# CUHK-SE-Group/MicroRank

Measured on AMD Instinct MI355X. Metric: PageRank GTEPS + RCA windows ranked/sec at 1/2/4/8 MI355X; % HBM roofline, higher is better.
Workload: dtype f64

## Files before the change

### microrank_amd/csrc/mr_graph_build.hip

```cpp
#include <algorithm>
#include <cstring>
#include <vector>

#include "mr_detect_dev.h"
#include "mr_prim.h"
#include "mr_sort.h"

namespace {
constexpr int BT = 256;
constexpr int LDS_HIST = 8192;
constexpr int ESET = 1024;
constexpr uint64_t EMPTY = ~0ull;

__device__ __forceinline__ uint64_t hmix(uint64_t z) {
    z ^= z >> 33;
    z *= 0xff51afd7ed558ccdull;
    z ^= z >> 33;
    z *= 0xc4ceb9fe1a85ec53ull;
    return z ^ (z >> 33);
}

__global__ void k_count_codes(const int64_t* span, int64_t S, int32_t* cnt) {
    int64_t i = (int64_t)blockIdx.x * blockDim.x + threadIdx.x;
    if (i < S) atomicAdd(&cnt[span[i]], 1);
// ... 1814 lines not shown
        }
    }
    if (i < w.n_po) {
        const int32_t t = w.po_tr[i], op = w.po_op[i];
        const int sd = side_of(w.state[t]);
        if (sd >= 0) w.o.g[sd].rs_ops[w.x.g[sd].zoff[t] + (i - w.po_off[t])] = w.o.g[sd].node_of_code[op];
    }
}

int mr_ix_launch2_batch(mr_ctx* ctx, int n, const mr_spans* const* sps, uint8_t* const* d_states, mr_graph* const* g0s,
                        mr_graph* const* g1s, IxBuild* const* b0s, IxBuild* const* b1s, int64_t* const* d_outs,
                        const DetIn* dets, bool fuse) {
    if (n < 1 || n > IXW || getenv("MR_NO_IX2") != nullptr) return MR_ERR_STATE;
    for (int k = 0; k < n; ++k) {
        const mr_spans* sp = sps[k];
        if (!sp->ekey.p || sp->n_podops > NS_PMAX || 2 * (3 * (int64_t)sp->n_podops + sp->n_edge_keys) > IX_LDS_WORDS)
            return MR_ERR_STATE;
    }
    hipStream_t st = ctx->stream;
    IxBatch<IxWinSel> as{};
    IxBatch<IxWinStats> at{};
    const char* ee = getenv("MR_IX_EPT");
    const int ept = ee ? std::max(1, atoi(ee)) : IX_EPT;
    IxBatch<IxWinCross> ac{};
    IxBatch<IxWinNodes> an{};
    IxBatch<IxWinTraces> ar{};
    as.n = at.n = ac.n = an.n = ar.n = n;
    int32_t bs = 0, bt = 0, bc = 0, br = 0;
    size_t lds = 4;
    int64_t words = 0;
    std::vector<int64_t> woff((size_t)n);
    const int TP = fuse ? DB : SEL_TILE;
    for (int k = 0; k < n; ++k) {
        const mr_spans* sp = sps[k];
        const int32_t NT = sp->n_traces, NP = sp->n_podops;
        const int64_t nek = sp->n_edge_keys;
        IxSide2 xs;
        NsArgs2 na;
        TrOut2 to;
        IxBuild* b[2] = {b0s[k], b1s[k]};
        mr_graph* g[2] = {g0s[k], g1s[k]};
        for (int j = 0; j < 2; ++j) {
            IxBuild& B = *b[j];
            mr_graph* G = g[j];
            B.dense = true;
            B.small = true;
            B.ecap = (uint64_t)nek;
            B.gkp = sp->ekey.p;
            MR_TRY(B.tflag.alloc(ctx, std::max(NT, 1)));
            MR_TRY(B.tpos.alloc(ctx, (size_t)NT + 1));
            MR_TRY(B.zoff.alloc(ctx, (size_t)NT + 1));
            MR_TRY(B.ocnt.alloc(ctx, std::max(NP, 1)));
            MR_TRY(B.ofirst.alloc(ctx, std::max(NP, 1)));
            MR_TRY(B.ocov.alloc(ctx, std::max(NP, 1)));
            MR_TRY(B.gc.alloc(ctx, (size_t)std::max<int64_t>(nek, 1)));
            MR_TRY(B.node_of_code.alloc(ctx, std::max(NP, 1)));
            MR_TRY(G->node_podop.alloc(ctx, std::max(NP, 1)));
            MR_TRY(G->len_o.alloc(ctx, std::max(NP, 1)));
            MR_TRY(G->nchild.alloc(ctx, std::max(NP, 1)));
            MR_TRY(G->cov.alloc(ctx, std::max(NP, 1)));
            MR_TRY(G->ss_par.alloc(ctx, NS_EMAX));
            MR_TRY(G->ss_off.alloc(ctx, (size_t)NP + 1));
            MR_TRY(G->trace_code.alloc(ctx, std::max(NT, 1)));
            MR_TRY(G->len_t.alloc(ctx, std::max(NT, 1)));
            MR_TRY(G->rs_ops.alloc(ctx, (size_t)std::max<int64_t>(sp->n_po, 1)));
            MR_TRY(G->rs_off.alloc(ctx, (size_t)NT + 1));
            xs.g[j] = IxSide{B.tflag.p, B.ocnt.p, B.ofirst.p, B.ocov.p, B.tpos.p, B.zoff.p, B.gc.p};
            na.g[j] = NsArgs{B.gc.p, B.ocnt.p, B.ofirst.p, B.ocov.p, B.node_of_code.p, G->node_podop.p, G->len_o.p,
                             G->nchild.p, G->cov.p, G->ss_par.p, G->ss_off.p, B.tpos.p + NT, B.zoff.p + NT, G->rs_off.p,
                             d_outs[k] + 8 * j, nullptr, nullptr};
            to.g[j] = TrOut{G->trace_code.p, G->len_t.p, G->rs_ops.p, G->rs_off.p, B.node_of_code.p};
        }
        const int32_t nt = (int32_t)std::max<int64_t>(cdiv((int64_t)NT, TP), 1);
        woff[(size_t)k] = words;
        words += 4 * (int64_t)nt;
        as.b0[k] = bs;
        bs += nt;
        as.w[k] = IxWinSel{dets ? dets[k] : DetIn{}, d_states[k], sp->tlen.p, sp->po_off.p, nullptr, nek, NT, NP, xs};
        at.b0[k] = bt;
        const int64_t ne = std::max(sp->n_po, sp->n_ed);
        const int ek = ee ? ept : ne >= IX_EPT_BIG ? IX_EPT_BATCH : IX_EPT;
        if (NT) bt += std::max(1, std::min(256, cdiv(ne, (int64_t)IX_BT * ek)));
        lds = std::max(lds, 2 * (3 * (size_t)NP + (size_t)nek) * sizeof(int32_t));
        at.w[k] = IxWinStats{d_states[k], sp->po_tr.p, sp->po_op.p, sp->po_cnt.p, sp->po_first.p, sp->ed_tr.p, sp->ed_eid.p,
                             sp->ed_cnt.p, sp->n_po, sp->n_ed, NP, (int32_t)nek, xs};
        ac.b0[k] = bc;
        bc += (int32_t)cdiv(sp->n_xj, 256);
        ac.w[k] = IxWinCross{d_states[k], sp->xj_tc.p, sp->xj_tp.p, sp->xj_eid.p, sp->n_xj, xs};
        an.b0[k] = 2 * k;
        an.w[k] = IxWinNodes{sp->ekey.p, nek, NP, 0, na};
        ar.b0[k] = br;
        if (NT || sp->n_po) br += (int32_t)cdiv(std::max<int64_t>(NT, sp->n_po), 256);
        ar.w[k] = IxWinTraces{d_states[k], sp->tlen.p, sp->po_tr.p, sp->po_op.p, sp->po_off.p, sp->n_po, NT, 0, xs, to};
    }
    for (int k = n; k <= IXW; ++k) {
        if (k <= IXW) {
            as.b0[k] = bs;
            at.b0[k] = bt;
            ac.b0[k] = bc;
            an.b0[k] = 2 * n;
            ar.b0[k] = br;
        }
    }
    unsigned long long* dst = nullptr;
    uint64_t epoch = 0;
    MR_TRY(mr_dl_status(ctx, words, &dst, &epoch));
    for (int k = 0; k < n; ++k) as.w[k].st = dst + woff[(size_t)k];
    if (fuse) {
        hipLaunchKernelGGL(k_ix_detect_scan2_b, dim3(bs), dim3(DB), 0, st, as, epoch);
    } else {
        if (dets) {
            int32_t bd = 0;
            IxBatch<IxWinSel> ad = as;
            for (int k = 0; k < n; ++k) {
                ad.b0[k] = bd;
                bd += (int32_t)cdiv((int64_t)sps[k]->n_traces, DB);
            }
            for (int k = n; k <= IXW; ++k) ad.b0[k] = bd;
            if (bd) hipLaunchKernelGGL(k_ix_detect_b, dim3(bd), dim3(DB), 0, st, ad);
        }
        hipLaunchKernelGGL(k_ix_sel_scan2_b, dim3(bs), dim3(SEL_T), 0, st, as, epoch);
    }
    if (bt) hipLaunchKernelGGL(k_ix_stats2_b, dim3(bt), dim3(IX_BT), lds, st, at);
    if (bc) hipLaunchKernelGGL(k_ix_cross2_b, dim3(bc), dim3(256), 0, st, ac);
    hipLaunchKernelGGL(k_nodes_small2_b, dim3(2 * n), dim3(NS_T), 0, st, an);
    if (br) hipLaunchKernelGGL(k_ix_traces2_b, dim3(br), dim3(256), 0, st, ar);
    MR_TRY_HIP(ctx, hipGetLastError());
    return MR_OK;
}

constexpr int LB_T = 512;
constexpr int64_t LB_LDS_WORDS = 30720;
constexpr int32_t LB_A3MAX = 4096;
bool mr_lo_fits(const mr_spans* sp) {
    return sp->indexed && sp->ekey.p && sp->n_podops <= NS_PMAX && sp->n_edge_keys <= NS_EMAX &&
           2 * (3 * (int64_t)sp->n_podops + sp->n_edge_keys) + 2 * (int64_t)sp->n_svcops <= LB_LDS_WORDS &&
           sp->n_svcops <= LB_A3MAX && sp->n_traces <= (1 << 24);
}
struct IxWinLoB {
    const int32_t *lo_tr, *lo_len, *lo_kid, *lo_first, *bstart;
    const int64_t *lo_off, *lsv_off, *le_off;
    const uint16_t *lo16, *lo_cnt;
    const uint32_t *lsv, *le;
    const long long *lo_ts, *lo_te, *lo_mx;
    const double* a3;
    const uint8_t* a3v;
    int64_t t0, t1;
    uint8_t* state;
    int8_t* side;
    unsigned long long* counts;
    int32_t NT, NP, nek, nsvc;
    uint32_t* kcnt[2];
    int64_t* tot[2];
    uint32_t* rows;
};
__host__ __device__ __forceinline__ size_t lo_region0(size_t gbytes) {
    return 2 * gbytes > (size_t)2048 * 8 ? 2 * gbytes : (size_t)2048 * 8;
}
constexpr int LB_R = 4;
__device__ __forceinline__ int32_t lo_trace_of(uint32_t e, uint32_t n, const uint32_t* st, int32_t nt) {
    if (n > 0) return (int32_t)(e / n);
    int32_t lo = 0;
#pragma unroll
    for (int32_t step = LO_BT_MAX / 2; step >= 1; step >>= 1) {
        const int32_t mid = lo + step;
        lo = mid < nt && st[mid] <= e ? mid : lo;
    }
    return lo;
}
__global__ void __launch_bounds__(LB_T, 6) k_lo_build_b(IxBatch<IxWinLoB> a) {
    extern __shared__ __attribute__((aligned(16))) unsigned char lraw[];
    __shared__ uint32_t pst[LO_BT_MAX + 1], est[LO_BT_MAX + 1];
    __shared__ int8_t ss[LO_BT_MAX];
    __shared__ unsigned long long bc[5][LB_T / WAVE];
    const int k = ixb_pick(a.b0, a.n);
    const IxWinLoB& w = a.w[k];
    const int32_t blk = (int32_t)blockIdx.x - a.b0[k];
    const int tid = threadIdx.x, lane = tid & (WAVE - 1), wv = tid / WAVE;
    const int32_t NP = w.NP, nek = w.nek;
    const size_t gbytes = ((size_t)NP * 12 + (size_t)nek * 4 + 15) / 16 * 16;
    const size_t reg0 = lo_region0(gbytes);
    double* la3 = (double*)(lraw + reg0);
    double* prod = (double*)lraw;
    const uint32_t cap = (uint32_t)(reg0 / 8 / LB_T * LB_T);
    for (int32_t c = tid; c < w.nsvc; c += LB_T) la3[c] = w.a3v[c] ? w.a3[c] : 0.0;
    const int32_t T0 = w.bstart[blk], nt = w.bstart[blk + 1] - T0;
    const int64_t P0 = w.lo_off[T0], Q0 = w.le_off[T0], V0 = w.lsv_off[T0];
    const uint32_t np = (uint32_t)(w.lo_off[T0 + nt] - P0), nq = (uint32_t)(w.le_off[T0 + nt] - Q0);
    const uint32_t nv = (uint32_t)(w.lsv_off[T0 + nt] - V0);
    if (tid == 0) {
        pst[nt] = np;
        est[nt] = nq;
    }
    constexpr int NS = LO_BT_MAX / LB_T;
    uint32_t va[NS], vb[NS];
    bool act[NS];
    double expect[NS];
    long long mx[NS];
    unsigned long long rows = 0;
#pragma unroll
    for (int q = 0; q < NS; ++q) {
        const int32_t t = q * LB_T + tid;
        const bool valid = t < nt;
        const int64_t i = (int64_t)T0 + (valid ? t : nt - 1);
        const int32_t len = w.lo_len[i];
        const long long ts = w.lo_ts[i], te = w.lo_te[i];
        mx[q] = w.lo_mx[i];
        va[q] = (uint32_t)(w.lsv_off[i] - V0);
        vb[q] = (uint32_t)(w.lsv_off[i + 1] - V0);
        const bool in = valid && len > 0 && ts >= w.t0 && te <= w.t1;
        rows += in ? (unsigned long long)len : 0ull;
        act[q] = in && mx[q] > 0;
        expect[q] = 0.0;
    }
    __syncthreads();
    for (uint32_t r0 = 0; r0 < nv; r0 += cap) {
        const uint32_t rn = min(cap, nv - r0);
        constexpr int LU = 8;
        for (uint32_t x0 = 0; x0 < rn; x0 += LU * LB_T) {
            uint32_t v[LU];
#pragma unroll
            for (int u = 0; u < LU; ++u) {
                const uint32_t x = x0 + (uint32_t)(u * LB_T + tid);
                v[u] = w.lsv[V0 + (int64_t)(r0 + min(x, rn - 1))];
            }
#pragma unroll
            for (int u = 0; u < LU; ++u) {
                const uint32_t x = x0 + (uint32_t)(u * LB_T + tid);
                if (x < rn) prod[x] = (double)(v[u] >> 16) * la3[v[u] & 0xffffu];
            }
        }
        __syncthreads();
#pragma unroll
        for (int q = 0; q < NS; ++q)
            if (act[q]) {
                const uint32_t lo = max(va[q], r0), hi = min(vb[q], r0 + rn);
                for (uint32_t j = lo; j < hi; j += 8) {
                    double p8[8];
#pragma unroll
                    for (int u = 0; u < 8; ++u) p8[u] = prod[min(j + u, hi - 1) - r0];
#pragma unroll
                    for (int u = 0; u < 8; ++u)
                        if (j + u < hi) expect[q] += p8[u];
                }
            }
        __syncthreads();
    }
    for (size_t x = (size_t)tid * 4; x < reg0; x += (size_t)LB_T * 4) *(uint32_t*)(lraw + x) = 0u;
    unsigned long long nab = 0, nno = 0, nz0 = 0, nz1 = 0;
#pragma unroll
    for (int q = 0; q < NS; ++q) {
        const int32_t t = q * LB_T + tid;
        const bool valid = t < nt;
        const int64_t i = (int64_t)T0 + (valid ? t : nt - 1);
        const int32_t kid0 = w.lo_kid[i], tr = w.lo_tr[i];
        const int64_t pa = w.lo_off[i], pb = w.lo_off[i + 1], ea = w.le_off[i];
        const int stt = act[q] ? ((double)mx[q] / 1000.0 > expect[q] ? 2 : 1) : 0;
        const int s_ = valid ? (stt == 2 ? 0 : stt == 1 ? 1 : -1) : -1;
        if (valid) {
            w.state[tr] = (uint8_t)stt;
            w.side[i] = (int8_t)s_;
            ss[t] = (int8_t)s_;
            pst[t] = (uint32_t)(pa - P0);
            est[t] = (uint32_t)(ea - Q0);
        }
        nab += stt == 2;
        nno += stt == 1;
        if (s_ == 0) nz0 += (unsigned long long)(pb - pa);
        else if (s_ == 1) nz1 += (unsigned long long)(pb - pa);
        const int kid = valid ? kid0 : -1;
        const int kp = __shfl_up(kid, 1, WAVE);
        const bool hd = kid >= 0 && (lane == 0 || kp != kid);
        const unsigned long long H = __ballot(hd), B0 = __ballot(s_ == 0), B1 = __ballot(s_ == 1);
        if (hd) {
            const unsigned long long above = lane == WAVE - 1 ? 0ull : H & (~0ull << (lane + 1));
            const unsigned long long run = (above ? (above & (0ull - above)) - 1ull : ~0ull) & (~0ull << lane);
            const uint32_t c0 = (uint32_t)__popcll(B0 & run), c1 = (uint32_t)__popcll(B1 & run);
            if (c0) atomicAdd(&w.kcnt[0][kid], c0);
            if (c1) atomicAdd(&w.kcnt[1][kid], c1);
        }
    }
    __syncthreads();
    constexpr int LB_LANE = 8;
    const bool lanewise = nt > 0 && pst[nt] - pst[nt - 1] <= (uint32_t)LB_LANE;
    if (lanewise) {
#pragma unroll
        for (int q = 0; q < NS; ++q) {
            const int32_t t = q * LB_T + tid;
            const int sd = t < nt ? (int)ss[t] : -1;
            if (sd < 0) continue;
            unsigned char* G = lraw + (size_t)sd * gbytes;
            const uint32_t a0 = pst[t], n = pst[t + 1] - a0, rot = n ? (uint32_t)t % n : 0u;
            uint32_t pc[LB_LANE];
            int32_t fr[LB_LANE];
#pragma unroll
            for (int u = 0; u < LB_LANE; ++u) {
                const uint32_t j = (uint32_t)u + rot;
                const int64_t e = P0 + (int64_t)a0 + (u < (int)n ? (j >= n ? j - n : j) : 0u);
                pc[u] = (uint32_t)w.lo16[e] | ((uint32_t)w.lo_cnt[e] << 16);
                fr[u] = w.lo_first[e];
            }
#pragma unroll
            for (int u = 0; u < LB_LANE; ++u)
                if (u < (int)n) {
                    const uint32_t c = pc[u] & 0xffffu;
                    atomicAdd((unsigned long long*)G + c, (unsigned long long)(pc[u] >> 16) | (1ull << 32));
                    atomicMax((int32_t*)(G + (size_t)NP * 8) + c, 0x7fffffff - fr[u]);
                }
            const uint32_t b0e = est[t], m = est[t + 1] - b0e, rte = m ? (uint32_t)t % m : 0u;
            uint32_t* Ge = (uint32_t*)(G + (size_t)NP * 12);
            for (uint32_t u0 = 0; u0 < m; u0 += LB_LANE) {
                uint32_t ev[LB_LANE];
#pragma unroll
                for (int u = 0; u < LB_LANE; ++u) {
                    const uint32_t j = u0 + (uint32_t)u, jr = j + rte;
                    ev[u] = w.le[Q0 + (int64_t)b0e + (j < m ? (jr >= m ? jr - m : jr) : 0u)];
                }
#pragma unroll
                for (int u = 0; u < LB_LANE; ++u)
                    if (u0 + (uint32_t)u < m) atomicAdd(Ge + (ev[u] & 0xffffu), ev[u] >> 16);
            }
        }
    }
    const uint32_t n0 = nt ? pst[1 < nt ? 1 : nt] - pst[0] : 0u;
    const uint32_t npo = n0 > 0 && np == (uint32_t)nt * n0 ? n0 : 0u;
    constexpr int NW = LB_T / WAVE;
    const uint32_t nmax = lanewise ? 0u : max(np, nq);
    for (uint32_t b0 = (uint32_t)wv * (LB_R * WAVE); b0 < nmax; b0 += NW * LB_R * WAVE) {
        uint32_t pc[LB_R], ev[LB_R];
        int32_t fr[LB_R];
#pragma unroll
        for (int r = 0; r < LB_R; ++r) {
            const uint32_t o = b0 + (uint32_t)(r * WAVE + lane);
            if (b0 < np) {
                const int64_t e = P0 + (int64_t)min(o, np - 1u);
                pc[r] = (uint32_t)w.lo16[e] | ((uint32_t)w.lo_cnt[e] << 16);
                fr[r] = w.lo_first[e];
            }
            if (b0 < nq) ev[r] = w.le[Q0 + (int64_t)min(o, nq - 1u)];
        }
#pragma unroll
        for (int r = 0; r < LB_R; ++r) {
            const uint32_t o = b0 + (uint32_t)(r * WAVE + lane);
            if (o < np) {
                const int sd = ss[lo_trace_of(o, npo, pst, nt)];
                if (sd >= 0) {
                    unsigned char* G = lraw + (size_t)sd * gbytes;
                    const uint32_t c = pc[r] & 0xffffu;
                    atomicAdd((unsigned long long*)G + c, (unsigned long long)(pc[r] >> 16) | (1ull << 32));
                    atomicMax((int32_t*)(G + (size_t)NP * 8) + c, 0x7fffffff - fr[r]);
                }
            }
            if (o < nq) {
                const int sd = ss[lo_trace_of(o, 0u, est, nt)];
                if (sd >= 0)
                    atomicAdd((uint32_t*)(lraw + (size_t)sd * gbytes + (size_t)NP * 12) + (ev[r] & 0xffffu), ev[r] >> 16);
            }
        }
    }
    __syncthreads();
    {
        unsigned long long v[5] = {nab, nno, rows, nz0, nz1};
#pragma unroll
        for (int m = 32; m >= 1; m >>= 1)
#pragma unroll
            for (int q = 0; q < 5; ++q) v[q] += __shfl_xor(v[q], m, WAVE);
        if (lane == 0)
#pragma unroll
            for (int q = 0; q < 5; ++q) bc[q][wv] = v[q];
    }
    __syncthreads();
    if (tid < 5) {
        unsigned long long v = 0;
        for (int q = 0; q < NW; ++q) v += bc[tid][q];
        if (v) {
            if (tid < 3) atomicAdd(&w.counts[(size_t)(blk % CSH) * 3 + tid], v);
            else atomicAdd((unsigned long long*)&w.tot[tid - 3][1], v);
        }
    }
    const size_t rw = 3 * (size_t)NP + (size_t)nek;
    uint32_t* R = w.rows + (size_t)blk * 2 * rw;
    for (int g = 0; g < 2; ++g) {
        const unsigned char* G = lraw + (size_t)g * gbytes;
        uint32_t* Rg = R + (size_t)g * rw;
        for (int32_t c = tid; c < NP; c += LB_T) {
            const unsigned long long v = ((const unsigned long long*)G)[c];
            Rg[c] = (uint32_t)v;
            Rg[NP + c] = (uint32_t)(v >> 32);
            Rg[2 * NP + c] = ((const uint32_t*)(G + (size_t)NP * 8))[c];
        }
        for (int32_t x = tid; x < nek; x += LB_T) Rg[3 * NP + x] = ((const uint32_t*)(G + (size_t)NP * 12))[x];
    }
    __syncthreads();
}
constexpr int LP_T = 256, LP_I = 16, LP_TILE = LP_T * LP_I;
struct IxWinLoPos {
    const int8_t* side;
    int32_t NT, pad_;
    unsigned long long* st;
    int32_t* pinv[2];
    int64_t* tot[2];
};
__global__ void __launch_bounds__(LP_T) k_lo_pos_b(IxBatch<IxWinLoPos> a, uint64_t epoch) {
    __shared__ int32_t sa[2][LP_T];
    __shared__ int32_t ex[2];
    __shared__ int32_t so[2][LP_TILE];
    const int k = ixb_pick(a.b0, a.n);
    const IxWinLoPos& w = a.w[k];
    const int32_t blk = (int32_t)blockIdx.x - a.b0[k], nblk = a.b0[k + 1] - a.b0[k];
    const int tid = threadIdx.x, lane = tid & (WAVE - 1);
    const int64_t base = (int64_t)blk * LP_TILE + (int64_t)tid * LP_I;
    int8_t sd[LP_I];
    if (base + LP_I <= w.NT) {
        const uint4 v = *(const uint4*)(w.side + base);
        memcpy(sd, &v, 16);
    } else {
#pragma unroll
        for (int q = 0; q < LP_I; ++q) sd[q] = base + q < w.NT ? w.side[base + q] : (int8_t)-1;
    }
    int32_t c0 = 0, c1 = 0;
#pragma unroll
    for (int q = 0; q < LP_I; ++q) {
        c0 += sd[q] == 0;
        c1 += sd[q] == 1;
    }
    sa[0][tid] = c0;
    sa[1][tid] = c1;
    __syncthreads();
    for (int o = 1; o < LP_T; o <<= 1) {
        const int32_t v0 = tid >= o ? sa[0][tid - o] : 0, v1 = tid >= o ? sa[1][tid - o] : 0;
        __syncthreads();
        sa[0][tid] += v0;
        sa[1][tid] += v1;
        __syncthreads();
    }
    if (tid < 2 * WAVE) {
        const int g = tid / WAVE;
        const int32_t agg = sa[g][LP_T - 1];
        const int64_t e = dl_lookback_wave(w.st + (size_t)g * nblk, blk, agg, epoch);
        if (lane == 0) {
            ex[g] = (int32_t)e;
            if (blk == nblk - 1) w.tot[g][0] = e + agg;
        }
    }
    int32_t r0 = sa[0][tid] - c0, r1 = sa[1][tid] - c1;
#pragma unroll
    for (int q = 0; q < LP_I; ++q) {
        const int32_t ix = (int32_t)(base + q);
        if (sd[q] == 0) so[0][r0++] = ix;
        else if (sd[q] == 1) so[1][r1++] = ix;
    }
    __syncthreads();
    for (int g = 0; g < 2; ++g) {
        const int32_t n = sa[g][LP_T - 1], e = ex[g];
        for (int32_t x = tid; x < n; x += LP_T) w.pinv[g][e + x] = so[g][x];
    }
}
struct IxLoRed {
    const uint32_t* rows;
    int32_t nblk, NP, nek, pad_;
    int32_t *ocnt[2], *ofinv[2], *ocov[2];
    uint32_t* gc[2];
};
__global__ void __launch_bounds__(256) k_lo_reduce_b(IxBatch<IxLoRed> a) {
    const int k = ixb_pick(a.b0, a.n);
    const IxLoRed& w = a.w[k];
    const int64_t rw = 3 * (int64_t)w.NP + w.nek;
    const int64_t col = (int64_t)((int32_t)blockIdx.x - a.b0[k]) * 256 + threadIdx.x;
    if (col >= 2 * rw) return;
    const int g = (int)(col / rw);
    const int64_t c = col - (int64_t)g * rw;
    const bool mx = c >= 2 * (int64_t)w.NP && c < 3 * (int64_t)w.NP;
    const uint32_t* p = w.rows + col;
    const size_t stride = 2 * (size_t)rw;
    uint32_t acc = 0;
    int32_t b = 0;
    for (; b + 8 <= w.nblk; b += 8) {
        uint32_t v[8];
#pragma unroll
        for (int q = 0; q < 8; ++q) v[q] = p[(size_t)(b + q) * stride];
#pragma unroll
        for (int q = 0; q < 8; ++q) acc = mx ? max(acc, v[q]) : acc + v[q];
    }
    for (; b < w.nblk; ++b) {
        const uint32_t v = p[(size_t)b * stride];
        acc = mx ? max(acc, v) : acc + v;
    }
    const int32_t NP = w.NP;
    if (c < NP) w.ocnt[g][c] = (int32_t)acc;
    else if (c < 2 * (int64_t)NP) w.ocov[g][c - NP] = (int32_t)acc;
    else if (c < 3 * (int64_t)NP) w.ofinv[g][c - 2 * NP] = (int32_t)acc;
    else w.gc[g][c - 3 * NP] = acc;
}

int64_t mr_lo_zero_words(const mr_spans* sp) {
    return 2 * ((int64_t)std::max(sp->lo_nk, 1) + 3 * (int64_t)sp->n_podops + std::max<int64_t>(sp->n_edge_keys, 1));
}
int mr_lo_launch_batch(mr_ctx* ctx, int n, const mr_spans* const* sps, mr_graph* const* g0s, mr_graph* const* g1s,
                       IxBuild* const* b0s, IxBuild* const* b1s, int64_t* const* d_outs, const DetIn* dets,
                       uint32_t* const* zw) {
    if (n < 1 || n > IXW || getenv("MR_NO_IX2") != nullptr) return MR_ERR_STATE;
    for (int k = 0; k < n; ++k)
        if (!sps[k]->lo_ok || !mr_lo_fits(sps[k])) return MR_ERR_STATE;
    hipStream_t st = ctx->stream;
    IxBatch<IxWinLoB> ab{};
    IxBatch<IxLoRed> ar{};
    IxBatch<IxWinLoPos> ap{};
    IxBatch<IxWinCross> ac{};
    IxBatch<IxWinNodes> an{};
    ab.n = ar.n = ap.n = ac.n = an.n = n;
    int32_t bb = 0, bc = 0, br = 0, bp = 0;
    int64_t rwords = 0, sbytes = 0;
    std::vector<int64_t> roff((size_t)n), soff((size_t)n);
    size_t lds = 4;
    int64_t words = 0;
    std::vector<int64_t> woff((size_t)n);
    for (int k = 0; k < n; ++k) {
        const mr_spans* sp = sps[k];
        const int32_t NT = sp->n_traces, NP = sp->n_podops;
        const int64_t nek = sp->n_edge_keys, nk = std::max(sp->lo_nk, 1);
        IxSide2 xs;
        NsArgs2 na;
        IxBuild* b[2] = {b0s[k], b1s[k]};
        mr_graph* g[2] = {g0s[k], g1s[k]};
        IxWinLoB& L = ab.w[k];
        const int64_t per = nk + 3 * (int64_t)NP + std::max<int64_t>(nek, 1);
        for (int j = 0; j < 2; ++j) {
            IxBuild& B = *b[j];
            mr_graph* G = g[j];
            B.dense = true;
            B.small = true;
            B.ecap = (uint64_t)nek;
            B.gkp = sp->ekey.p;
            uint32_t* z = zw[k] + j * per;
            B.kcnt = z;
            int32_t* ocnt = (int32_t*)(z + nk);
            int32_t* ofinv = ocnt + NP;
            int32_t* ocov = ofinv + NP;
            uint32_t* gc = (uint32_t*)(ocov + NP);
            MR_TRY(B.pinv.alloc(ctx, std::max(NT, 1)));
            MR_TRY(B.node_of_code.alloc(ctx, std::max(NP, 1)));
            MR_TRY(G->node_podop.alloc(ctx, std::max(NP, 1)));
            MR_TRY(G->len_o.alloc(ctx, std::max(NP, 1)));
            MR_TRY(G->nchild.alloc(ctx, std::max(NP, 1)));
            MR_TRY(G->cov.alloc(ctx, std::max(NP, 1)));
            MR_TRY(G->u_o.alloc(ctx, std::max(NP, 1)));
            MR_TRY(G->pw.alloc(ctx, std::max(NP, 1)));
            MR_TRY(G->ss_par.alloc(ctx, NS_EMAX));
            MR_TRY(G->ss_off.alloc(ctx, (size_t)NP + 1));
            xs.g[j] = IxSide{nullptr, ocnt, ofinv, ocov, nullptr, nullptr, gc};
            int64_t* out = d_outs[k] + 8 * j;
            na.g[j] = NsArgs{gc, ocnt, ofinv, ocov, B.node_of_code.p, G->node_podop.p, G->len_o.p, G->nchild.p, G->cov.p,
                             G->ss_par.p, G->ss_off.p, out + 5, out + 6, nullptr, out, G->u_o.p, G->pw.p, 1};
            ap.w[k].pinv[j] = B.pinv.p;
            ap.w[k].tot[j] = out + 5;
            L.kcnt[j] = B.kcnt;
            L.tot[j] = out + 5;
            IxLoRed& R = ar.w[k];
            R.ocnt[j] = ocnt;
            R.ofinv[j] = ofinv;
            R.ocov[j] = ocov;
            R.gc[j] = gc;
        }
        const int32_t nt = sp->lo_nblk;
        const int64_t rw = 3 * (int64_t)NP + nek;
        roff[(size_t)k] = rwords;
        rwords += (int64_t)nt * 2 * rw;
        ar.w[k].nblk = nt;
        ar.w[k].NP = NP;
        ar.w[k].nek = (int32_t)nek;
        ar.b0[k] = br;
        br += (int32_t)cdiv(2 * rw, 256);
        const int32_t npb = (int32_t)std::max<int64_t>(cdiv((int64_t)NT, LP_TILE), 1);
        woff[(size_t)k] = words;
        words += 2 * (int64_t)npb;
        ap.b0[k] = bp;
        bp += npb;
        ap.w[k].NT = NT;
        soff[(size_t)k] = sbytes;
        sbytes += ((int64_t)NT + 15) / 16 * 16;
        ab.b0[k] = bb;
        bb += nt;
        const DetIn& d = dets[k];
        L.bstart = sp->lo_bstart.p;
        L.lo_tr = sp->lo_tr.p;
        L.lo_len = sp->lo_len.p;
        L.lo_kid = sp->lo_kid.p;
        L.lo_first = sp->lo_first.p;
        L.lo_off = sp->lo_off.p;
        L.lsv_off = sp->lsv_off.p;
        L.le_off = sp->le_off.p;
        L.lo16 = sp->lo16.p;
        L.lo_cnt = sp->lo_cnt.p;
        L.lsv = sp->lsv.p;
        L.le = sp->le.p;
        L.lo_ts = sp->lo_ts.p;
        L.lo_te = sp->lo_te.p;
        L.lo_mx = sp->lo_mx.p;
        L.a3 = d.a3;
        L.a3v = d.a3v;
        L.t0 = d.t0;
        L.t1 = d.t1;
        L.state = d.state;
        L.counts = d.counts;
        L.NT = NT;
        L.NP = NP;
        L.nek = (int32_t)nek;
        L.nsvc = sp->n_svcops;
        lds = std::max(lds, lo_region0(((size_t)NP * 12 + (size_t)nek * 4 + 15) / 16 * 16) + (size_t)sp->n_svcops * 8);
        ac.b0[k] = bc;
        bc += (int32_t)cdiv(sp->n_xj, 256);
        ac.w[k] = IxWinCross{d.state, sp->xj_tc.p, sp->xj_tp.p, sp->xj_eid.p, sp->n_xj, xs};
        an.b0[k] = 2 * k;
        an.w[k] = IxWinNodes{sp->ekey.p, nek, NP, 0, na};
    }
    for (int k = n; k <= IXW; ++k) {
        ab.b0[k] = bb;
        ar.b0[k] = br;
        ap.b0[k] = bp;
        ac.b0[k] = bc;
        an.b0[k] = 2 * n;
    }
    unsigned long long* dst = nullptr;
    uint64_t epoch = 0;
    MR_TRY(mr_dl_status(ctx, words, &dst, &epoch));
    DBuf<uint32_t> rows;
    DBuf<int8_t> side;
    MR_TRY(rows.alloc(ctx, (size_t)std::max<int64_t>(rwords, 1)));
    MR_TRY(side.alloc(ctx, (size_t)std::max<int64_t>(sbytes, 16)));
    for (int k = 0; k < n; ++k) {
        ab.w[k].rows = rows.p + roff[(size_t)k];
        ar.w[k].rows = rows.p + roff[(size_t)k];
        ab.w[k].side = side.p + soff[(size_t)k];
        ap.w[k].side = side.p + soff[(size_t)k];
        ap.w[k].st = dst + woff[(size_t)k];
    }
    hipLaunchKernelGGL(k_lo_build_b, dim3(bb), dim3(LB_T), lds, st, ab);
    hipLaunchKernelGGL(k_lo_pos_b, dim3(bp), dim3(LP_T), 0, st, ap, epoch);
    hipLaunchKernelGGL(k_lo_reduce_b, dim3(br), dim3(256), 0, st, ar);
    if (bc) hipLaunchKernelGGL(k_ix_cross2_b, dim3(bc), dim3(256), 0, st, ac);
    hipLaunchKernelGGL(k_nodes_small2_b, dim3(2 * n), dim3(NS_T), 0, st, an);
    MR_TRY_HIP(ctx, hipGetLastError());
    return MR_OK;
}

int mr_ix_launch(mr_ctx* ctx, const mr_spans* sp, const uint8_t* d_mask, mr_graph* g, IxBuild& b, int64_t* d_out) {
    return ix_launch(ctx, sp, d_mask, g, b, d_out, false);
}
int mr_ix_finish(mr_ctx* ctx, const mr_spans* sp, mr_graph* g, IxBuild& b, const int64_t* h) {
    MR_TRY(ix_finish(ctx, sp, g, b, h, false));
    return mr_graph_post_build(ctx, g);
}
int mr_ix_finish_unprepared(mr_ctx* ctx, const mr_spans* sp, mr_graph* g, IxBuild& b, const int64_t* h) {
    MR_TRY(ix_finish(ctx, sp, g, b, h, false));
    g->rs_is_sr = true;
    g->pr_identity = true;
    g->n_pr = g->T;
    return MR_OK;
}

int mr_graph_post_build(mr_ctx* ctx, mr_graph* g) {
    g->rs_is_sr = true;
    g->pr_identity = true;
    g->n_pr = g->T;
    PhaseTimer pt(ctx->stream, "prepare");
    MR_TRY(mr_graph_prepare(ctx, g));
    pt.mark("done");
    return MR_OK;
}

int mr_graph_build_dev(mr_ctx* ctx, const mr_spans* sp, const uint8_t* d_mask, mr_graph** out, const int64_t* win) {
    auto g = new mr_graph();
    g->ctx = ctx;
    static const bool no_index = getenv("MR_NO_INDEX") != nullptr;
    const bool indexed = sp->indexed && !no_index && (!win || sp->uniform_times);
    int rc = indexed ? graph_build_indexed(ctx, sp, d_mask, g) : graph_build_rows(ctx, sp, d_mask, win, g);
    if (rc == MR_OK) rc = mr_graph_post_build(ctx, g);
    if (rc != MR_OK) {
        delete g;
        return rc;
    }
    *out = g;
    return MR_OK;
}

extern "C" int mr_graph_build(mr_ctx* ctx, const mr_spans* sp, const uint8_t* trace_mask, mr_graph** out) {
    if (!ctx || !sp || !trace_mask || !out || sp->ctx != ctx) return mr_fail(ctx, MR_ERR_ARG, "mr_graph_build: bad arguments");
    MR_TRY_HIP(ctx, hipSetDevice(ctx->device));
    DBuf<uint8_t> mask;
    MR_TRY(mask.upload(ctx, trace_mask, (size_t)sp->n_traces));
    MR_TRY(mr_graph_build_dev(ctx, sp, mask.p, out, nullptr));
    mr_handle_add(ctx, *out, [](void* h) { delete (mr_graph*)h; });
    return MR_OK;
}

extern "C" int mr_graph_build_sharded(mr_ctx* ctx, const mr_spans* sp, const uint8_t* trace_mask, mr_graph** out) {
    if (!ctx || !sp || !trace_mask || !out || sp->ctx != ctx)
        return mr_fail(ctx, MR_ERR_ARG, "mr_graph_build_sharded: bad arguments");
    if (!mr_coll_ready(ctx) && ctx->nranks != 1) return mr_fail(ctx, MR_ERR_COMM, "no collective backend");
    if (!sp->indexed) return mr_fail(ctx, MR_ERR_STATE, "span table has no per-trace index (sharded build needs it)");
    MR_TRY_HIP(ctx, hipSetDevice(ctx->device));
    *out = nullptr;
    DBuf<uint8_t> mask;
    MR_TRY(mask.upload(ctx, trace_mask, (size_t)sp->n_traces));
    auto g = new mr_graph();
    g->ctx = ctx;
    int rc = graph_build_indexed(ctx, sp, mask.p, g, true);
    if (rc == MR_OK) {
        g->rs_is_sr = true;
        g->pr_identity = true;
        g->n_pr = g->T;
        rc = mr_graph_prepare(ctx, g);
    }
    if (rc == MR_OK) rc = hipStreamSynchronize(ctx->stream) == hipSuccess ? MR_OK : mr_fail(ctx, MR_ERR_HIP, "sync");
    if (rc != MR_OK) {
        delete g;
        return rc;
    }
    mr_handle_add(ctx, g, [](void* h) { delete (mr_graph*)h; });
    *out = g;
    return MR_OK;
}

extern "C" int mr_graph_nodes(const mr_graph* g, int32_t* node_podop, int32_t* trace_code) {
    if (!g) return MR_ERR_ARG;
    mr_ctx* ctx = g->ctx;
    if (!g->node_podop.p && g->N) return mr_fail(ctx, MR_ERR_STATE, "graph was not built from spans");
    if (node_podop && g->N) MR_TRY(g->node_podop.download(ctx, node_podop, g->N));
    if (trace_code && g->T) MR_TRY(g->trace_code.download(ctx, trace_code, g->T));
    MR_TRY_HIP(ctx, hipStreamSynchronize(ctx->stream));
    return MR_OK;
}

extern "C" int mr_graph_export(const mr_graph* g, int64_t* sr_off, int32_t* sr_ops, int32_t* len_t, int32_t* len_o,
                               int64_t* ss_off, int32_t* ss_par, int32_t* nchild) {
    if (!g) return MR_ERR_ARG;
    mr_ctx* ctx = g->ctx;
    if (sr_off) MR_TRY(g->rs_off.download(ctx, sr_off, (size_t)g->T + 1));
    if (sr_ops) MR_TRY(g->rs_ops.download(ctx, sr_ops, (size_t)g->nnz_rs));
    if (sr_ops) {
        std::vector<int64_t> off((size_t)g->T + 1);
        MR_TRY(g->rs_off.download(ctx, off.data(), off.size()));
        MR_TRY_HIP(ctx, hipStreamSynchronize(ctx->stream));
        for (int32_t t = 0; t < g->T; ++t) std::sort(sr_ops + off[t], sr_ops + off[t + 1]);
    }
    if (len_t) MR_TRY(g->len_t.download(ctx, len_t, (size_t)g->T));
    if (len_o) MR_TRY(g->len_o.download(ctx, len_o, (size_t)g->N));
    if (ss_off) MR_TRY(g->ss_off.download(ctx, ss_off, (size_t)g->N + 1));
    if (ss_par) MR_TRY(g->ss_par.download(ctx, ss_par, (size_t)g->E));
    if (nchild) MR_TRY(g->nchild.download(ctx, nchild, (size_t)g->N));
    MR_TRY_HIP(ctx, hipStreamSynchronize(ctx->stream));
    return MR_OK;
}
```

### microrank_amd/csrc/mr_pagerank.hip

```cpp
#include <algorithm>
#include <chrono>
#include <cmath>
#include <cstdlib>
#include <cstring>
#include <memory>
#include <queue>
#include <type_traits>

#include "mr_internal.h"
#include "mr_prim.h"
#include "mr_sort.h"

namespace {

constexpr int TB = 256;
constexpr int LDS_NODES = 8192;
constexpr int VCAP = 2048;
constexpr int LONG_PAIR = 32;
constexpr int TSHIFT_MIN = 8, TSHIFT_MAX = 12;

__device__ __forceinline__ uint64_t mix64(uint64_t z) {
    z += 0x9E3779B97F4A7C15ull;
    z = (z ^ (z >> 30)) * 0xBF58476D1CE4E5B9ull;
    z = (z ^ (z >> 27)) * 0x94D049BB133111EBull;
// ... 1253 lines not shown
    if (i < N) {
        G.sp0[i] = v0;
        G.su0[i] = (double)G.u_o[G.perm ? G.perm[i] : i] * v0;
    }
    if (i >= N && i < N + TR_PAD) G.su0[i] = G.su1[i] = 0.0;
    if (i < T) {
        const double q = (double)G.w_tq[i] * v0;
        if (G.fp32) G.q32[i] = (float)q; else G.q64[i] = q;
    }
    if (i < MSLOT_WORDS) G.mslot[i] = i < 2 * MSH ? d2bits(1.0) : 0ull;
}
__global__ void __launch_bounds__(KB) k_kind_insert_b(const SDev* __restrict__ sd, int32_t ng, uint64_t seed,
                                                      uint64_t hmask) {
    const SDev& G = sd[sd_graph(sd, ng, (int32_t)blockIdx.x, 1)];
    kind_insert_body<false, 2>((int32_t)blockIdx.x - G.b_kins, G.off, nullptr, G.o16, G.w_t, G.T, G.hk, G.cr,
                                  G.slot_of, (uint64_t)(G.cap - 1), seed, nullptr, hmask);
}
__global__ void k_kind_verify_b(const SDev* __restrict__ sd, int32_t ng) {
    const SDev& G = sd[sd_graph(sd, ng, (int32_t)blockIdx.x, 2)];
    const int32_t t = ((int32_t)blockIdx.x - G.b_kver) * blockDim.x + threadIdx.x;
    if (t >= G.T) return;
    const KCnt ks = G.cr[G.slot_of[t]];
    const int32_t r = ks.rep;
    G.kind[t] = (double)ks.cnt;
    if (r == t) return;
    const int64_t a0 = G.off[t], a1 = G.off[t + 1], b0 = G.off[r], b1 = G.off[r + 1];
    bool eq = (a1 - a0) == (b1 - b0);
    if (eq && a1 > a0) eq = __float_as_uint(G.w_t[t]) == __float_as_uint(G.w_t[r]);
    for (int64_t i = 0; eq && i < a1 - a0; ++i) eq = G.o16[a0 + i] == G.o16[b0 + i];
    if (!eq) atomicOr(G.flag, 1);
}
__global__ void k_pref_partial_b(const SDev* __restrict__ sd, int32_t ng) {
    __shared__ double red[TB / WAVE];
    const SDev& G = sd[sd_graph(sd, ng, (int32_t)blockIdx.x, 3)];
    const int32_t blk = (int32_t)blockIdx.x - G.b_pref;
    double a = 0.0, b = 0.0;
    const int32_t i = blk * blockDim.x + threadIdx.x;
    if (i < G.T) {
        const int32_t ln = G.len_t[i];
        a = 1.0 / G.kind[i];
        if (ln == 0) atomicOr(G.flag + 1, 1);
        b = ln ? 1.0 / (double)ln : 0.0;
    }
    a = block_sum(a, red);
    b = block_sum(b, red);
    if (threadIdx.x == 0) {
        G.ppart[2 * blk] = a;
        G.ppart[2 * blk + 1] = b;
    }
}
__global__ void k_pref_total_b(const SDev* __restrict__ sd) {
    __shared__ double red[1024 / WAVE];
    const SDev& G = sd[blockIdx.x];
    const int32_t nb = cdiv_d(G.T, TB);
    double a = 0.0, b = 0.0;
    for (int32_t i = threadIdx.x; i < nb; i += blockDim.x) {
        a += G.ppart[2 * i];
        b += G.ppart[2 * i + 1];
    }
    a = block_sum(a, red);
    b = block_sum(b, red);
    if (threadIdx.x == 0) {
        G.scal[2] = a;
        G.scal[3] = b;
    }
}
__global__ void k_pref_apply_b(const SDev* __restrict__ sd, int32_t ng) {
    const SDev& G = sd[sd_graph(sd, ng, (int32_t)blockIdx.x, 3)];
    const int32_t t = ((int32_t)blockIdx.x - G.b_pref) * blockDim.x + threadIdx.x;
    if (t >= G.T) return;
    const int32_t i = G.tpos[t];
    const double k = G.kind[t];
    double v;
    if (!G.anomaly) v = 1.0 / k / G.scal[2];
    else v = 1.0 / (k / G.scal[2] * G.phi + 1.0 / (double)G.len_t[t]) / G.scal[3] * G.phi;
    const float vf = (float)v;
    G.pref[t] = vf;
    G.c_t[t] = G.cd * vf;
    G.c_tp[i] = G.cd * vf;
}

constexpr int LO_NOC_MAX = 4096;
struct LDev {
    int32_t T, N, W, anomaly, fp32, NP;
    int32_t b_cs, n_cs, b_fill, nbp, b_app;
    int64_t st_off;
    float cd;
    double phi, v0;
    const int32_t* pinv;
    const int64_t* lo_off;
    const uint16_t* lo16;
    const int32_t *lo_len, *lo_kid, *noc;
    const uint32_t* kcnt;
    int64_t* c64;
    int32_t* coff;
    uint16_t* tids;
    float *w_tp, *c_tp;
    double* kind;
    int32_t* lenp;
    uint8_t* trun;
    double *ppart, *scal;
    int32_t* flag;
    unsigned long long* mslot;
    double *sp0, *su0, *su1, *q64;
    float* q32;
    const float* u_o;
};
__device__ __forceinline__ int32_t ld_graph(const LDev* ld, int32_t n, int32_t blk, int which) {
    int32_t lo = 0, hi = n - 1;
    while (lo < hi) {
        const int32_t mid = (lo + hi + 1) >> 1;
        const LDev& g = ld[mid];
        const int32_t s0 = which == 0 ? g.b_cs : which == 1 ? g.b_fill : g.b_app;
        if (s0 <= blk) lo = mid; else hi = mid - 1;
    }
    return lo;
}
__global__ void __launch_bounds__(TS_T) k_lo_cs_b(const LDev* __restrict__ ld, int32_t n, unsigned long long* st,
                                                 uint64_t epoch) {
    const LDev& G = ld[ld_graph(ld, n, (int32_t)blockIdx.x, 0)];
    tr_chunk_scan_body((int32_t)blockIdx.x - G.b_cs, G.n_cs, G.pinv, G.lo_off, G.T, G.W, G.c64, G.coff, st + G.st_off,
                       epoch);
}
__global__ void __launch_bounds__(256) k_lo_fill_b(const LDev* __restrict__ ld, int32_t n) {
    __shared__ double red[256 / WAVE];
    __shared__ uint16_t lnoc[LO_NOC_MAX];
    const LDev& G = ld[ld_graph(ld, n, (int32_t)blockIdx.x, 1)];
    const int32_t blk = (int32_t)blockIdx.x - G.b_fill;
    const int64_t i = (int64_t)blk * 256 + threadIdx.x;
    const int32_t T = G.T, N = G.N;
    for (int32_t c = threadIdx.x; c < G.NP; c += 256) lnoc[c] = (uint16_t)G.noc[c];
    __syncthreads();
    double a = 0.0, b = 0.0;
    if (i < (int64_t)G.W * WAVE) {
        const int32_t k = (int32_t)(i / WAVE), lane = (int32_t)(i % WAVE);
        int64_t e0 = 0, len = 0, rot = 0;
        const int32_t ix = i < T ? G.pinv[i] : -1;
        const int32_t kid = i < T ? G.lo_kid[ix] : -1;
        const int32_t kp = __shfl_up(kid, 1, WAVE);
        const bool hd = lane == 0 || kid < 0 || kid != kp;
        const unsigned long long hm = __ballot(hd);
        const unsigned long long below = hm & (lane == WAVE - 1 ? ~0ull : (2ull << lane) - 1ull);
        const int32_t ixh = __shfl(ix, 63 - __builtin_clzll(below), WAVE);
        const bool mt = G.trun && G.c64[k + 1] - G.c64[k] <= MR_TR_TIERS512;
        if (i < T && G.trun) {
            const unsigned long long above = lane == WAVE - 1 ? 0ull : hm & (~0ull << (lane + 1));
            G.trun[i] = !mt ? (uint8_t)1 : hd ? (uint8_t)((above ? __builtin_ctzll(above) : WAVE) - lane) : (uint8_t)0;
        }
        if (i < T) {
            e0 = G.lo_off[ix];
            len = G.lo_off[ix + 1] - e0;
            rot = len ? (int64_t)((uint32_t)(mt ? ixh : ix) % (uint32_t)len) : 0;
            const int32_t L = G.lo_len[ix];
            const uint32_t kc = G.kcnt[G.lo_kid[ix]];
            G.w_tp[i] = L > 0 ? (float)(1.0 / (double)L) : 0.0f;
            G.lenp[i] = L;
            G.kind[i] = (double)kc;
            a = 1.0 / (double)kc;
            b = L ? 1.0 / (double)L : 0.0;
        }
        const int64_t nc = G.c64[k + 1] - G.c64[k];
        unsigned long long* dst = (unsigned long long*)G.tids + (size_t)G.c64[k] * WAVE + lane;
        constexpr int TF_CH = 4;
        for (int64_t c0 = 0; c0 < nc; c0 += TF_CH) {
            uint16_t idv[4 * TF_CH];
#pragma unroll
            for (int q = 0; q < 4 * TF_CH; ++q) {
                const int64_t e = 4 * c0 + q, jx = rot + e;
                idv[q] = e < len ? lnoc[G.lo16[e0 + (jx >= len ? jx - len : jx)]] : (uint16_t)(N + lane);
            }
#pragma unroll
            for (int u = 0; u < TF_CH; ++u)
                if (c0 + u < nc)
                    dst[(size_t)(c0 + u) * WAVE] = (unsigned long long)idv[4 * u] | (unsigned long long)idv[4 * u + 1] << 16 |
                                                   (unsigned long long)idv[4 * u + 2] << 32 |
                                                   (unsigned long long)idv[4 * u + 3] << 48;
        }
    }
    a = block_sum(a, red);
    b = block_sum(b, red);
    if (threadIdx.x == 0) {
        G.ppart[2 * blk] = a;
        G.ppart[2 * blk + 1] = b;
    }
}
__global__ void __launch_bounds__(1024) k_lo_total_b(const LDev* __restrict__ ld) {
    __shared__ double red[1024 / WAVE];
    const LDev& G = ld[blockIdx.x];
    double a = 0.0, b = 0.0;
    for (int32_t i = threadIdx.x; i < G.nbp; i += blockDim.x) {
        a += G.ppart[2 * i];
        b += G.ppart[2 * i + 1];
    }
    a = block_sum(a, red);
    b = block_sum(b, red);
    if (threadIdx.x == 0) {
        G.scal[2] = a;
        G.scal[3] = b;
    }
}
__global__ void k_lo_apply_b(const LDev* __restrict__ ld, int32_t n) {
    const LDev& G = ld[ld_graph(ld, n, (int32_t)blockIdx.x, 2)];
    const int64_t i = (int64_t)((int32_t)blockIdx.x - G.b_app) * blockDim.x + threadIdx.x;
    const int32_t T = G.T, N = G.N;
    const double v0 = G.v0;
    if (i < T) {
        const double k = G.kind[i];
        double v;
        if (!G.anomaly) v = 1.0 / k / G.scal[2];
        else v = 1.0 / (k / G.scal[2] * G.phi + 1.0 / (double)G.lenp[i]) / G.scal[3] * G.phi;
        const float vf = (float)v;
        G.c_tp[i] = G.cd * vf;
        const double q = (double)G.w_tp[i] * v0;
        if (G.fp32) G.q32[i] = (float)q; else G.q64[i] = q;
    }
    if (i < N) {
        G.sp0[i] = v0;
        G.su0[i] = (double)G.u_o[i] * v0;
    }
    if (i >= N && i < N + TR_PAD) G.su0[i] = G.su1[i] = 0.0;
    if (i < MSLOT_WORDS) G.mslot[i] = i < 2 * MSH ? d2bits(1.0) : 0ull;
    if (i < 4) G.flag[i] = 0;
    if (i < 8 && i != 2 && i != 3) G.scal[i] = 0.0;
}

__global__ void k_iter_init(const float* w_t, const double* mw, const float* u_o, int32_t N, int32_t T, int64_t T_all,
                            double* sp0, double* su0, double* su1, double* q64, float* q32, int fp32,
                            unsigned long long* mslot, const int32_t* perm) {
    int64_t i = (int64_t)blockIdx.x * blockDim.x + threadIdx.x;
    const double v0 = 1.0 / (double)((int64_t)N + T_all);
    if (i < N) {
        sp0[i] = v0;
        su0[i] = (double)u_o[perm ? perm[i] : i] * v0;
    }
    if (i >= N && i < N + TR_PAD) su0[i] = su1[i] = 0.0;
    if (i < T) {
        double q = (mw ? mw[i] : (double)w_t[i]) * v0;
        if (fp32) q32[i] = (float)q; else q64[i] = q;
    }
    if (i < MSLOT_WORDS) mslot[i] = i < 2 * MSH ? d2bits(1.0) : 0ull;
}
__global__ void k_pr_reset_init(int32_t T, int64_t cap, int32_t N, float* pref, float* c_t, unsigned long long* hk,
                                KCnt* cr, int32_t* flag, double* scal, const float* w_t, const double* mw,
                                const float* u_o, int64_t T_all, double* sp0, double* su0, double* su1, double* q64,
                                float* q32, int fp32, unsigned long long* mslot, const int32_t* perm, int su32,
                                float* suf0, float* suf1) {
    const int64_t i = (int64_t)blockIdx.x * blockDim.x + threadIdx.x;
    if (i < T) {
        pref[i] = 0.0f;
        c_t[i] = 0.0f;
    }
    if (i < cap) {
        hk[i] = 0ull;
        cr[i] = KCnt{0u, 0x7fffffff};
    }
    if (i < 8) flag[i] = 0;
    if (i < 8) scal[i] = 0.0;
    const double v0 = 1.0 / (double)((int64_t)N + T_all);
    if (i < N) {
        sp0[i] = v0;
        const double su = (double)u_o[perm ? perm[i] : i] * v0;
        su0[i] = su32 ? (double)(float)su : su;
        if (su32) suf0[i] = (float)su;
    }
    if (i >= N && i < N + TR_PAD) su0[i] = su1[i] = 0.0;
    if (su32 && i >= N && i < N + TR_PAD) suf0[i] = suf1[i] = 0.0f;
    if (i < T) {
        const double q = (mw ? mw[i] : (double)w_t[i]) * v0;
        if (fp32) q32[i] = (float)q; else q64[i] = q;
    }
    if (i < MSLOT_WORDS) mslot[i] = i < 2 * MSH ? d2bits(1.0) : 0ull;
}

struct GDev {
    const int64_t* rs_off;
    const int32_t* rs_ops;
    const uint16_t* rs16;
    const uint16_t* rsw;
    const int32_t* perm;
    int32_t n_hot;
    const uint16_t* tids;
    const int32_t* coff;
    const int32_t* wtile;
    const float* c_tp;
    const float* w_tp;
    const double* mw_tp;
    const uint8_t* hmask;
    const uint8_t* trun;
    const uint32_t* ctids;
    const int32_t* ccoff;
    int32_t nhr;
    int32_t hop[8];
    const float* c_t;
    const float* w_t;
    const float* u_o;
    const float* pw;
    const uint16_t* ltr;
    const int64_t* pr_beg;
    const int32_t* tile_pr0;
    const int32_t* lp;
    const int32_t* tile_lp0;
    const int32_t* op_pr_off;
    const int32_t* op_pr;
    const int64_t* ss_off;
    const int32_t* ss_par;
    void* q[2];
    double* sub[2];
// ... 3491 lines not shown
```

Baseline: 1075.

## Fold per-block row reduction into build kernel via global atomics

```diff
diff --git a/microrank_amd/csrc/mr_graph_build.hip b/microrank_amd/csrc/mr_graph_build.hip
--- a/microrank_amd/csrc/mr_graph_build.hip
+++ b/microrank_amd/csrc/mr_graph_build.hip
@@ -1990,7 +1990,8 @@
     int32_t NT, NP, nek, nsvc;
     uint32_t* kcnt[2];
     int64_t* tot[2];
-    uint32_t* rows;
+    int32_t *ocnt[2], *ofinv[2], *ocov[2];
+    uint32_t* gc[2];
 };
 __host__ __device__ __forceinline__ size_t lo_region0(size_t gbytes) {
     return 2 * gbytes > (size_t)2048 * 8 ? 2 * gbytes : (size_t)2048 * 8;
@@ -2011,9 +2012,11 @@
     __shared__ uint32_t pst[LO_BT_MAX + 1], est[LO_BT_MAX + 1];
     __shared__ int8_t ss[LO_BT_MAX];
     __shared__ unsigned long long bc[5][LB_T / WAVE];
-    const int k = ixb_pick(a.b0, a.n);
+    const int32_t gb = (int32_t)(gridDim.x - 1u - blockIdx.x);
+    int k = 0;
+    while (k + 1 < a.n && a.b0[k + 1] <= gb) ++k;
     const IxWinLoB& w = a.w[k];
-    const int32_t blk = (int32_t)blockIdx.x - a.b0[k];
+    const int32_t blk = gb - a.b0[k];
     const int tid = threadIdx.x, lane = tid & (WAVE - 1), wv = tid / WAVE;
     const int32_t NP = w.NP, nek = w.nek;
     const size_t gbytes = ((size_t)NP * 12 + (size_t)nek * 4 + 15) / 16 * 16;
@@ -2216,20 +2219,20 @@
             else atomicAdd((unsigned long long*)&w.tot[tid - 3][1], v);
         }
     }
-    const size_t rw = 3 * (size_t)NP + (size_t)nek;
-    uint32_t* R = w.rows + (size_t)blk * 2 * rw;
     for (int g = 0; g < 2; ++g) {
         const unsigned char* G = lraw + (size_t)g * gbytes;
-        uint32_t* Rg = R + (size_t)g * rw;
         for (int32_t c = tid; c < NP; c += LB_T) {
             const unsigned long long v = ((const unsigned long long*)G)[c];
-            Rg[c] = (uint32_t)v;
-            Rg[NP + c] = (uint32_t)(v >> 32);
-            Rg[2 * NP + c] = ((const uint32_t*)(G + (size_t)NP * 8))[c];
-        }
-        for (int32_t x = tid; x < nek; x += LB_T) Rg[3 * NP + x] = ((const uint32_t*)(G + (size_t)NP * 12))[x];
-    }
-    __syncthreads();
+            const int32_t f = ((const int32_t*)(G + (size_t)NP * 8))[c];
+            if ((uint32_t)v) atomicAdd(&w.ocnt[g][c], (int32_t)(uint32_t)v);
+            if (v >> 32) atomicAdd(&w.ocov[g][c], (int32_t)(v >> 32));
+            if (f > 0) atomicMax(&w.ofinv[g][c], f);
+        }
+        for (int32_t x = tid; x < nek; x += LB_T) {
+            const uint32_t e = ((const uint32_t*)(G + (size_t)NP * 12))[x];
+            if (e) atomicAdd(&w.gc[g][x], e);
+        }
+    }
 }
 constexpr int LP_T = 256, LP_I = 16, LP_TILE = LP_T * LP_I;
 struct IxWinLoPos {
@@ -2294,43 +2297,6 @@
         for (int32_t x = tid; x < n; x += LP_T) w.pinv[g][e + x] = so[g][x];
     }
 }
-struct IxLoRed {
-    const uint32_t* rows;
-    int32_t nblk, NP, nek, pad_;
-    int32_t *ocnt[2], *ofinv[2], *ocov[2];
-    uint32_t* gc[2];
-};
-__global__ void __launch_bounds__(256) k_lo_reduce_b(IxBatch<IxLoRed> a) {
-    const int k = ixb_pick(a.b0, a.n);
-    const IxLoRed& w = a.w[k];
-    const int64_t rw = 3 * (int64_t)w.NP + w.nek;
-    const int64_t col = (int64_t)((int32_t)blockIdx.x - a.b0[k]) * 256 + threadIdx.x;
-    if (col >= 2 * rw) return;
-    const int g = (int)(col / rw);
-    const int64_t c = col - (int64_t)g * rw;
-    const bool mx = c >= 2 * (int64_t)w.NP && c < 3 * (int64_t)w.NP;
-    const uint32_t* p = w.rows + col;
-    const size_t stride = 2 * (size_t)rw;
-    uint32_t acc = 0;
-    int32_t b = 0;
-    for (; b + 8 <= w.nblk; b += 8) {
-        uint32_t v[8];
-#pragma unroll
-        for (int q = 0; q < 8; ++q) v[q] = p[(size_t)(b + q) * stride];
-#pragma unroll
-        for (int q = 0; q < 8; ++q) acc = mx ? max(acc, v[q]) : acc + v[q];
-    }
-    for (; b < w.nblk; ++b) {
-        const uint32_t v = p[(size_t)b * stride];
-        acc = mx ? max(acc, v) : acc + v;
-    }
-    const int32_t NP = w.NP;
-    if (c < NP) w.ocnt[g][c] = (int32_t)acc;
-    else if (c < 2 * (int64_t)NP) w.ocov[g][c - NP] = (int32_t)acc;
-    else if (c < 3 * (int64_t)NP) w.ofinv[g][c - 2 * NP] = (int32_t)acc;
-    else w.gc[g][c - 3 * NP] = acc;
-}
-
 int64_t mr_lo_zero_words(const mr_spans* sp) {
     return 2 * ((int64_t)std::max(sp->lo_nk, 1) + 3 * (int64_t)sp->n_podops + std::max<int64_t>(sp->n_edge_keys, 1));
 }
@@ -2342,14 +2308,13 @@
         if (!sps[k]->lo_ok || !mr_lo_fits(sps[k])) return MR_ERR_STATE;
     hipStream_t st = ctx->stream;
     IxBatch<IxWinLoB> ab{};
-    IxBatch<IxLoRed> ar{};
     IxBatch<IxWinLoPos> ap{};
     IxBatch<IxWinCross> ac{};
     IxBatch<IxWinNodes> an{};
-    ab.n = ar.n = ap.n = ac.n = an.n = n;
-    int32_t bb = 0, bc = 0, br = 0, bp = 0;
-    int64_t rwords = 0, sbytes = 0;
-    std::vector<int64_t> roff((size_t)n), soff((size_t)n);
+    ab.n = ap.n = ac.n = an.n = n;
+    int32_t bb = 0, bc = 0, bp = 0;
+    int64_t sbytes = 0;
+    std::vector<int64_t> soff((size_t)n);
     size_t lds = 4;
     int64_t words = 0;
     std::vector<int64_t> woff((size_t)n);
@@ -2394,21 +2359,12 @@
             ap.w[k].tot[j] = out + 5;
             L.kcnt[j] = B.kcnt;
             L.tot[j] = out + 5;
-            IxLoRed& R = ar.w[k];
-            R.ocnt[j] = ocnt;
-            R.ofinv[j] = ofinv;
-            R.ocov[j] = ocov;
-            R.gc[j] = gc;
+            L.ocnt[j] = ocnt;
+            L.ofinv[j] = ofinv;
+            L.ocov[j] = ocov;
+            L.gc[j] = gc;
         }
         const int32_t nt = sp->lo_nblk;
-        const int64_t rw = 3 * (int64_t)NP + nek;
-        roff[(size_t)k] = rwords;
-        rwords += (int64_t)nt * 2 * rw;
-        ar.w[k].nblk = nt;
-        ar.w[k].NP = NP;
-        ar.w[k].nek = (int32_t)nek;
-        ar.b0[k] = br;
-        br += (int32_t)cdiv(2 * rw, 256);
         const int32_t npb = (int32_t)std::max<int64_t>(cdiv((int64_t)NT, LP_TILE), 1);
         woff[(size_t)k] = words;
         words += 2 * (int64_t)npb;
@@ -2454,7 +2410,6 @@
     }
     for (int k = n; k <= IXW; ++k) {
         ab.b0[k] = bb;
-        ar.b0[k] = br;
         ap.b0[k] = bp;
         ac.b0[k] = bc;
         an.b0[k] = 2 * n;
@@ -2462,20 +2417,15 @@
     unsigned long long* dst = nullptr;
     uint64_t epoch = 0;
     MR_TRY(mr_dl_status(ctx, words, &dst, &epoch));
-    DBuf<uint32_t> rows;
     DBuf<int8_t> side;
-    MR_TRY(rows.alloc(ctx, (size_t)std::max<int64_t>(rwords, 1)));
     MR_TRY(side.alloc(ctx, (size_t)std::max<int64_t>(sbytes, 16)));
     for (int k = 0; k < n; ++k) {
-        ab.w[k].rows = rows.p + roff[(size_t)k];
-        ar.w[k].rows = rows.p + roff[(size_t)k];
         ab.w[k].side = side.p + soff[(size_t)k];
         ap.w[k].side = side.p + soff[(size_t)k];
         ap.w[k].st = dst + woff[(size_t)k];
     }
     hipLaunchKernelGGL(k_lo_build_b, dim3(bb), dim3(LB_T), lds, st, ab);
     hipLaunchKernelGGL(k_lo_pos_b, dim3(bp), dim3(LP_T), 0, st, ap, epoch);
-    hipLaunchKernelGGL(k_lo_reduce_b, dim3(br), dim3(256), 0, st, ar);
     if (bc) hipLaunchKernelGGL(k_ix_cross2_b, dim3(bc), dim3(256), 0, st, ac);
     hipLaunchKernelGGL(k_nodes_small2_b, dim3(2 * n), dim3(NS_T), 0, st, an);
     MR_TRY_HIP(ctx, hipGetLastError());
diff --git a/microrank_amd/csrc/mr_pagerank.hip b/microrank_amd/csrc/mr_pagerank.hip
--- a/microrank_amd/csrc/mr_pagerank.hip
+++ b/microrank_amd/csrc/mr_pagerank.hip
@@ -1429,7 +1429,7 @@
             len = G.lo_off[ix + 1] - e0;
             rot = len ? (int64_t)((uint32_t)(mt ? ixh : ix) % (uint32_t)len) : 0;
             const int32_t L = G.lo_len[ix];
-            const uint32_t kc = G.kcnt[G.lo_kid[ix]];
+            const uint32_t kc = G.kcnt[kid];
             G.w_tp[i] = L > 0 ? (float)(1.0 / (double)L) : 0.0f;
             G.lenp[i] = L;
             G.kind[i] = (double)kc;
```

Result: no change. 1089 (median of 5 runs) (+1.3%).
